# Hagtaril/HiddenPose

Hardware: AMD Instinct MI355X
Metric: samples/sec (128x128x512 meas) fwd+bwd (higher is better)
Workload: dtype f32; 1 GPU; NlosPose train step (fwd+L2Joint+BCEDice loss+bwd+Adam), 128x128x512 transients, batch 4/GPU, fp32, random-init weights, weight gradients of the 3^3 / 4^3 convolutions (and of small 1^3 ones) on a second stream; global_batch=4, world_size=1, parallelism=dp1

## Files before the change

### hiddenpose_amd/_lib.py

```python
from __future__ import annotations

import ctypes as C
import os
import threading

_PKG = os.path.dirname(os.path.abspath(__file__))
LIB_PATH = os.path.join(_PKG, "libhiddenpose_hip.so")

_lock = threading.Lock()
_lib = None


class HiddenPoseHipError(RuntimeError):
    pass


_vp, _fp, _i, _sz, _d = C.c_void_p, C.c_void_p, C.c_int, C.c_size_t, C.c_double
SIGNATURES = {
    "hp_version": (_i, []),
    "hp_last_error_string": (C.c_char_p, []),
    "hp_profile_enable": (_i, [_i]),
    "hp_profile_reset": (_i, []),
    "hp_profile_count": (_i, []),
    "hp_profile_get": (_i, [_i, C.c_char_p, _i, C.POINTER(C.c_int64), C.POINTER(C.c_double)]),
# ... 7 lines not shown
    "hp_lct_plan_create_mode": (_i, [C.POINTER(_vp), _i, _i, _d, _d, _i, _i, _i]),
    "hp_lct_plan_destroy": (_i, [_vp]),
    "hp_laplacian5_forward": (_i, [_fp, _fp, _fp, C.c_long, _i, _i, _i, _vp]),
    "hp_laplacian5_backward": (_i, [_fp, _fp, _fp, C.c_long, _i, _i, _i, _vp]),
    "hp_lct_workspace_bytes": (_sz, [_vp, _i]),
    "hp_lct_forward": (_i, [_vp, _fp, _fp, _i, _vp, _sz, _vp]),
    "hp_lct_backward": (_i, [_vp, _fp, _fp, _i, _vp, _sz, _vp]),
    "hp_lct_plan_get_invpsf": (_i, [_vp, _vp, _vp]),
    "hp_conv3d_packed_weight_elems": (_sz, [_vp]),
    "hp_conv3d_pack_weight": (_i, [_vp, _fp, _fp, _fp, _vp]),
    "hp_conv3d_unpack_wgrad": (_i, [_vp, _fp, _fp, _vp]),
    "hp_conv3d_forward": (_i, [_vp, _fp, _fp, _fp, _fp, _vp, _vp]),
    "hp_conv3d_backward_data": (_i, [_vp, _fp, _fp, _fp, _fp, _vp]),
    "hp_conv3d_backward_data_masked": (_i, [_vp, _fp, _fp, _fp, _fp, _vp, _vp]),
    "hp_conv3d_backward_data_bnsums": (_i, [_vp, _fp, _fp, _fp, _fp, _vp, _fp, _fp, _fp, _fp, _fp, _i, _vp, _vp, C.POINTER(C.c_int), _vp]),
    "hp_bn_backward_presummed": (_i, [_fp, _fp, _fp, C.c_long, _i, _fp, _fp, _fp, _fp, _i, _i, _fp, _fp, _vp, _vp, _vp, _i, _vp]),
    "hp_conv3d_backward_weight": (_i, [_vp, _fp, _fp, _fp, _vp]),
    "hp_conv3d_backward_weight_split": (_i, [_vp, C.POINTER(C.c_long), C.POINTER(C.c_long)]),
    "hp_bn_train_finalize": (_i, [_vp, C.c_long, _i, C.c_float, C.c_float, _fp, _fp, _fp, _fp, _vp]),
    "hp_bn_train_finalize_counted": (_i, [_vp, C.c_long, _i, C.c_float, C.c_float, _fp, _fp, _fp, _fp, _vp, _vp]),
    "hp_bn_eval_stats": (_i, [_fp, _fp, _i, C.c_float, _fp, _fp, _vp]),
    "hp_bn_apply": (_i, [_fp, _fp, _fp, C.c_long, _i, _fp, _fp, _fp, _fp, _i, _vp, _i, _vp]),
    "hp_bn_apply_res_bn": (_i, [_fp, _fp, _fp, C.c_long, _i, _fp, _fp, _fp, _fp, _i, _vp, _fp, _fp, _fp, _fp, _i, _vp]),
    "hp_cast_f32_to_bf16": (_i, [_fp, _vp, C.c_long, _vp]),
    "hp_cast_bf16_to_f32": (_i, [_vp, _fp, C.c_long, _vp]),
    "hp_bn_backward_workspace_bytes": (_sz, [_i]),
    "hp_bn_backward_dual": (_i, [_fp, _vp, C.c_long, _i, _fp, _fp, _fp, _fp, _fp, _i, _fp, _fp, _fp, _fp, _fp, _fp, _fp, _i,
                                 _fp, _fp, _vp, _i, _vp]),
    "hp_bn_backward": (_i, [_fp, _fp, _fp, _fp, _fp, C.c_long, _i, _fp, _fp, _fp, _fp, _i, _i, _fp, _fp, _vp, _vp, _i, _vp]),
    "hp_maxpool3d_k3s2_forward": (_i, [_fp, _fp, _i, _i, _i, _i, _i, _vp]),
# ... 194 lines not shown
```

### hiddenpose_amd/csrc/conv_kernels.hip

```cpp
#include <algorithm>
#include <cstdlib>
#include <cstring>
#include <mutex>
#include <type_traits>
#include <vector>

#include "hp_internal.h"

namespace hp {

using f32x16 = __attribute__((ext_vector_type(16))) float;
using bf16x8 = __attribute__((ext_vector_type(8))) __bf16;
using bf16x4 = __attribute__((ext_vector_type(4))) __bf16;
using bf16x2 = __attribute__((ext_vector_type(2))) __bf16;
using f32x2 = __attribute__((ext_vector_type(2))) float;
using s16x4 = __attribute__((ext_vector_type(4))) short;

__device__ __forceinline__ bf16x4 to_bf16x4(const float4 v) {
  const bf16x2 lo = __builtin_convertvector((f32x2){v.x, v.y}, bf16x2);
  const bf16x2 hi = __builtin_convertvector((f32x2){v.z, v.w}, bf16x2);
  return (bf16x4){lo[0], lo[1], hi[0], hi[1]};
}

enum IgemmMode { MODE_CONV = 0, MODE_DECONV = 1, MODE_DGRAD_S2K3 = 2, MODE_STEM = 3 };
// ... 27 lines not shown
    x = (int)(u & (unsigned)(g.gw - 1));
    y = (int)((u >> g.sw) & (unsigned)(g.gh - 1));
    z = (int)((u >> (g.sw + g.sh)) & (unsigned)(g.gd - 1));
    b = (int)(u >> (g.sw + g.sh + g.sd));
  } else {
    long t = m;
    x = (int)(t % g.gw);
    t /= g.gw;
    y = (int)(t % g.gh);
    t /= g.gh;
    z = (int)(t % g.gd);
    b = (int)(t / g.gd);
  }
}

template <int NP>
__device__ __forceinline__ void split_bf16(const float4 v, bf16x4 (&out)[NP]) {
  float4 r = v;
#pragma unroll
  for (int p = 0; p < NP; ++p) {
    out[p] = to_bf16x4(r);
    if (p + 1 < NP) {
      r.x -= (float)out[p][0];
      r.y -= (float)out[p][1];
      r.z -= (float)out[p][2];
      r.w -= (float)out[p][3];
    }
  }
}
template <int NP>
// ... 60 lines not shown
    dx = pw ? 1 - jw : 0;
    widx = (kd * 3 + kh) * 3 + kw;
  }
}

template <int BN>
struct TileCfg {
  static constexpr int WN = BN >= 64 ? 2 : 1;
  static constexpr int WM = 4 / WN;
  static constexpr int TM = BM / (WM * 32);
  static constexpr int TN = BN / (WN * 32);
};

__device__ __attribute__((aligned(256))) unsigned int g_zero_row[64];

template <int BN, bool STEM, bool STATS, int NP, bool XH = false, bool GL = false, bool BL = false, int BNS = 0>
__global__ __launch_bounds__(CT, (NP == 0 && BN == 128) ? 3 : 1) void k_igemm(const void* __restrict__ Xv, const float* __restrict__ Wp,
                                              const float* __restrict__ bias, void* __restrict__ Y,
                                              double* __restrict__ stats, const void* __restrict__ addend,
                                              const unsigned char* __restrict__ amask, IgemmGeom g) {
  const float* const X = (const float*)Xv;
  constexpr bool IOH = NP == 1;
  auto ld_x4 = [&](long off) -> float4 {
    if constexpr (IOH) return hp_ld4(Xv, off, g.xh);
    else return *(const float4*)(X + off);
  };
  auto ld_a4 = [&](long off) -> float4 {
    if constexpr (IOH) return hp_ld4(addend, off, g.ah);
    else return *(const float4*)((const float*)addend + off);
  };
  auto ld_a1 = [&](long off) -> float {
// ... 2 lines not shown
  };
  auto st_y4 = [&](long off, float4 v) {
    if constexpr (IOH) hp_st4(Y, off, v, g.yh);
    else *(float4*)((float*)Y + off) = v;
  };
  auto st_y1 = [&](long off, float v) {
    if constexpr (IOH) hp_st1(Y, off, v, g.yh);
    else ((float*)Y)[off] = v;
  };
  using C = TileCfg<BN>;
  constexpr bool BF = NP > 0;
  constexpr int NPL = NP > 0 ? NP : 1;
  static_assert(!XH || (NP == 1 && !STEM), "bf16-storage tiles: single bf16 plane, not the stem");
  static_assert(!GL || (XH && BN >= 64), "direct-to-LDS tiles: bf16 storage, 64 or 128 columns");
  static_assert(!BL || (!XH && !STEM), "buffer-load tiles: fp32 tensors in memory (any arithmetic), not the stem");
  constexpr int BKT = XH ? 64 : BK;
  constexpr int LDX = GL ? BKT : BKT + 8;
  constexpr int EPL = XH ? 8 : 4;
  constexpr int ARENA0 = (BM + BN) * LDK > NP * (BM + BN) * LDH / 2 ? (BM + BN) * LDK : NP * (BM + BN) * LDH / 2;
  constexpr int ARENA1 = XH && (BM + BN) * LDX / 2 > ARENA0 ? (BM + BN) * LDX / 2 : ARENA0;
  constexpr int GLBUF = (BM + BN) * 64;
  constexpr int ARENA = GL ? GLBUF : ARENA1;
  __shared__ __attribute__((aligned(16))) float smem[ARENA];
  float* const As = smem;
  float* const Bs = smem + BM * LDK;
  __bf16* const Ah = (__bf16*)smem;
  __bf16* const Bh = Ah + NPL * BM * (XH ? LDX : LDH);
  __shared__ float red[STATS ? 2 * BN * C::WM : 1];
  const int tid = threadIdx.x, lane = tid & 63, wave = tid >> 6;
  const int wm = wave / C::WN, wn = wave % C::WN;
  const int cls = blockIdx.z;
  unsigned mt_idx = blockIdx.x, nt_idx = blockIdx.y;
  if (g.tn > 0) {
    const unsigned i = blockIdx.x >> 3;
    nt_idx = i % (unsigned)g.tn;
    mt_idx = g.slab > 0 ? (blockIdx.x & 7u) * (unsigned)g.slab + i / (unsigned)g.tn : (i / (unsigned)g.tn) * 8u + (blockIdx.x & 7u);
    if ((long)mt_idx * BM >= g.M) return;
  } else if (g.slab > 0) {
    mt_idx = (blockIdx.x & 7u) * (unsigned)g.slab + (blockIdx.x >> 3);
    if ((long)mt_idx * BM >= g.M) return;
  }
  const long m0 = (long)mt_idx * BM;
  const int n0 = nt_idx * BN;
  const int pd = (cls >> 2) & 1, ph = (cls >> 1) & 1, pw = cls & 1;

  const int kq0 = tid & 7, r0 = tid >> 3;
  const int kq = GL ? (kq0 ^ ((r0 >> 1) & 7)) : kq0;
  int rb[4], rz[4], ry[4], rx[4];
  bool rv[4];
#pragma unroll
  for (int i = 0; i < 4; ++i) {
    const long m = m0 + r0 + 32 * i;
    rv[i] = m < g.M;
    grid_coords(g, rv[i] ? m : 0, rb[i], rz[i], ry[i], rx[i]);
    rx[i] *= g.s;
    ry[i] *= g.s;
    rz[i] *= g.s;
  }
  const int ntaps = STEM ? 1 : class_ntaps(g, cls);
  const int kpt = XH ? (g.Cin + BKT - 1) / BKT : g.kpt;
  const int KT = ntaps * kpt;

  long rowoff[4], wrow[BN / 32];
  unsigned long long vmask[4];
  bool wvalid[BN / 32];
#pragma unroll
  for (int i = 0; i < 4; ++i) {
    rowoff[i] = ((((long)rb[i] * g.Di + rz[i]) * g.Hi + ry[i]) * g.Wi + rx[i]) * g.Cin + kq * EPL;
    vmask[i] = 0ull;
  }
  if constexpr (!STEM) {
    for (int t = ntaps - 1; t >= 0; --t) {
      int dz, dy, dx, widx;
      tap_info(g, cls, t, dz, dy, dx, widx);
#pragma unroll
      for (int i = 0; i < 4; ++i) {
        const bool ok = rv[i] && (unsigned)(rz[i] + dz) < (unsigned)g.Di && (unsigned)(ry[i] + dy) < (unsigned)g.Hi &&
                        (unsigned)(rx[i] + dx) < (unsigned)g.Wi;
        vmask[i] = (vmask[i] << 1) | (ok ? 1ull : 0ull);
      }
    }
  }
#pragma unroll
  for (int i = 0; i < BN / 32; ++i) {
    const int n = n0 + r0 + 32 * i;
    wvalid[i] = n < g.Nout;
    const int nsrc = g.geglu ? ((n & 64) ? (g.Nout >> 1) + ((n >> 7) << 6) + (n & 63) : ((n >> 7) << 6) + (n & 63)) : n;
    wrow[i] = (long)nsrc * g.Cin + kq * EPL;
  }

  constexpr unsigned OOB = 0x80000000u;
  long rowbase = 0;
  unsigned xrow32[4] = {0u, 0u, 0u, 0u}, xvoff[4] = {OOB, OOB, OOB, OOB}, wvoff[BN / 32];
  long min_xoff = 0;
  if constexpr (BL) {
    for (int t = 0; t < ntaps; ++t) {
      int dz, dy, dx, widx;
      tap_info(g, cls, t, dz, dy, dx, widx);
      const long xo = (((long)dz * g.Hi + dy) * g.Wi + dx) * g.Cin;
      min_xoff = (t == 0 || xo < min_xoff) ? xo : min_xoff;
    }
    int b0, z0, y0, x0;
    grid_coords(g, m0 < g.M ? m0 : 0, b0, z0, y0, x0);
    rowbase = ((((long)b0 * g.Di + z0 * g.s) * g.Hi + y0 * g.s) * g.Wi + x0 * g.s) * g.Cin;
#pragma unroll
    for (int i = 0; i < 4; ++i) xrow32[i] = rv[i] ? (unsigned)((rowoff[i] - rowbase) * 4) : OOB;
#pragma unroll
    for (int i = 0; i < BN / 32; ++i) wvoff[i] = wvalid[i] ? (unsigned)(wrow[i] * 4) : OOB;
  }
  const __amdgpu_buffer_rsrc_t xrs = __builtin_amdgcn_make_buffer_rsrc(
      (void*)(X + (rowbase + min_xoff)), 0, hp_extent((long)g.B * g.Di * g.Hi * g.Wi * g.Cin, rowbase + min_xoff, 4), 0x00020000);
  const __amdgpu_buffer_rsrc_t wrs = __builtin_amdgcn_make_buffer_rsrc((void*)Wp, 0, hp_extent(g.welems, 0, 4), 0x00020000);
  float4 ra[4], rbw[BN / 32];
  uint4 ra8[XH ? 4 : 1];
  float4 rbw2[XH ? BN / 32 : 1];
  uint4 rb8[XH ? BN / 32 : 1];
  int ld_tap = 0, ld_ci = 0;
  long ld_xoff = 0, ld_woff = 0;
  unsigned ninv_lo[4] = {0u, 0u, 0u, 0u}, ninv_hi[4] = {0u, 0u, 0u, 0u};
// ... 4 lines not shown
      ninv_hi[i] = ~(unsigned)(vmask[i] >> 32);
    }
  }
  auto tap_offsets = [&](int t) {
    int dz, dy, dx, widx;
    tap_info(g, cls, t, dz, dy, dx, widx);
    ld_xoff = (((long)dz * g.Hi + dy) * g.Wi + dx) * g.Cin;
    ld_woff = (long)widx * g.Nout * g.Cin;
    if constexpr (BL) {
      const unsigned tb = (unsigned)t & 31u;
#pragma unroll
      for (int i = 0; i < 4; ++i)
        xvoff[i] = xrow32[i] | (__builtin_amdgcn_ubfe(t < 32 ? ninv_lo[i] : ninv_hi[i], tb, 1u) << 31);
    }
  };
  if (!STEM) tap_offsets(0);
  auto load_tile = [&](int kt) {
    if constexpr (STEM) {
      const int kbase = kt * BK + kq * 4;
#pragma unroll
      for (int i = 0; i < 4; ++i) {
        float v[4];
#pragma unroll
        for (int j = 0; j < 4; ++j) {
          const int kk = kbase + j;
          const int a = kk / 49, b = (kk / 7) % 7, c = kk % 7;
          const int z = rz[i] + a - 3, y = ry[i] + b - 3, x = rx[i] + c - 3;
          const bool ok = rv[i] && kk < 343 && (unsigned)z < (unsigned)g.Di && (unsigned)y < (unsigned)g.Hi &&
                          (unsigned)x < (unsigned)g.Wi;
          v[j] = ok ? X[(unsigned)(((rb[i] * g.Di + z) * g.Hi + y) * g.Wi + x)] : 0.f;
        }
// ... 34 lines not shown
        for (int i = 0; i < BN / 32; ++i) rbw[i] = __builtin_bit_cast(float4, __builtin_amdgcn_raw_buffer_load_b128(wrs, wvoff[i], ws, 0));
      } else {
#pragma unroll
        for (int i = 0; i < 4; ++i)
          ra[i] = (cok && (vmask[i] & 1ull)) ? ld_x4(xb + rowoff[i]) : make_float4(0, 0, 0, 0);
#pragma unroll
        for (int i = 0; i < BN / 32; ++i)
          rbw[i] = (cok && wvalid[i]) ? *(const float4*)(wb + wrow[i]) : make_float4(0, 0, 0, 0);
      }
      if (++ld_ci == kpt) {
        ld_ci = 0;
        if constexpr (!BL) {
#pragma unroll
          for (int i = 0; i < 4; ++i) vmask[i] >>= 1;
        }
        if (++ld_tap < ntaps) tap_offsets(ld_tap);
      }
    }
  };
  unsigned lds_a[4], lds_b[BN / 32];
#pragma unroll
  for (int i = 0; i < 4; ++i) {
    lds_a[i] = (unsigned)(((r0 + 32 * i) * LDK + kq * 4) * 4);
    asm volatile("" : "+v"(lds_a[i]));
  }
#pragma unroll
  for (int i = 0; i < BN / 32; ++i) {
    lds_b[i] = (unsigned)((BM * LDK + (r0 + 32 * i) * LDK + kq * 4) * 4);
    asm volatile("" : "+v"(lds_b[i]));
  }
  auto store_tile = [&]() {
// ... 180 lines not shown
      }
      __syncthreads();
    }
    if (kt + 1 < KT) {
      store_tile();
      __syncthreads();
    }
  }

  const bool dense_out = (g.os == 1 && g.gd == g.Do && g.gh == g.Ho && g.gw == g.Wo);
  if constexpr (BN >= 64) {
    constexpr int LDO = BN + 4, Q = BN / 4;
    static_assert(64 * LDO <= ARENA, "staging tile must fit the arena");
    static_assert(C::WM == 2 && C::TM == 2, "epilogue assumes 2 waves x 2 MFMA tiles along M");
    const bool vec_ok = (g.Nout & 3) == 0;
    const bool fast = !IOH && dense_out && vec_ok && m0 + BM <= g.M && n0 + BN <= g.Nout && !g.geglu;
    const long tile_el = m0 * g.Nout + n0;
    const long y_el = g.M * g.Nout;
    const unsigned y_rec = hp_extent(y_el, tile_el, 4);
    const __amdgpu_buffer_rsrc_t yrs = __builtin_amdgcn_make_buffer_rsrc((void*)((float*)Y + tile_el), 0, y_rec, 0x00020000);
    const __amdgpu_buffer_rsrc_t ars =
        __builtin_amdgcn_make_buffer_rsrc((void*)((addend ? (const float*)addend : (const float*)Y) + tile_el), 0, y_rec, 0x00020000);
    const __amdgpu_buffer_rsrc_t mrs = __builtin_amdgcn_make_buffer_rsrc(
        (void*)((amask ? amask : (const unsigned char*)Y) + (tile_el >> 2)), 0, hp_extent(y_el >> 2, tile_el >> 2, 1), 0x00020000);
    constexpr int RPK = CT / Q;
    const int r_l = tid / Q, q_l = tid % Q;
    const unsigned vo = (unsigned)((r_l * g.Nout + 4 * q_l) * 4);
    float4 bv = make_float4(0, 0, 0, 0);
    if (fast && bias) bv = *(const float4*)(bias + n0 + 4 * q_l);
    [[maybe_unused]] __amdgpu_buffer_rsrc_t zrs = yrs, bmrs = mrs;
    [[maybe_unused]] float4 b_m = make_float4(0, 0, 0, 0), b_r = b_m, b_sc = b_m, b_sh = b_m, b_s = b_m, b_d = b_m;
    if constexpr (BNS) {
      zrs = __builtin_amdgcn_make_buffer_rsrc((void*)(g.bn_z + tile_el), 0, y_rec, 0x00020000);
      if constexpr (BNS == 2)
        bmrs = __builtin_amdgcn_make_buffer_rsrc((void*)(g.bn_mask + (tile_el >> 2)), 0, hp_extent(y_el >> 2, tile_el >> 2, 1), 0x00020000);
      b_m = *(const float4*)(g.bn_mean + n0 + 4 * q_l);
      b_r = *(const float4*)(g.bn_rstd + n0 + 4 * q_l);
      if (BNS == 1 && g.bn_relu) {
        const float4 ga = *(const float4*)(g.bn_gamma + n0 + 4 * q_l), be = *(const float4*)(g.bn_beta + n0 + 4 * q_l);
        b_sc = make_float4(b_r.x * ga.x, b_r.y * ga.y, b_r.z * ga.z, b_r.w * ga.w);
        b_sh = make_float4(be.x - b_m.x * b_sc.x, be.y - b_m.y * b_sc.y, be.z - b_m.z * b_sc.z, be.w - b_m.w * b_sc.w);
      }
// ... 5 lines not shown
      for (int r = 0; r < 16; ++r) {
        const int rl = wm * 32 + (r & 3) + 8 * (r >> 2) + 4 * (lane >> 5);
#pragma unroll
        for (int j = 0; j < C::TN; ++j) smem[rl * LDO + wn * C::TN * 32 + j * 32 + (lane & 31)] = acc[h][j][r];
      }
      constexpr int K2 = (64 * Q) / CT;
      float4 avb[K2];
      unsigned mkb[K2];
      [[maybe_unused]] float4 zvb[BNS ? K2 : 1];
      [[maybe_unused]] unsigned bmb[BNS == 2 ? K2 : 1];
      if constexpr (BNS) {
#pragma unroll
        for (int k2 = 0; k2 < K2; ++k2) {
          const int rowc = k2 * RPK;
          const unsigned so = (unsigned)(((rowc >> 5) * (C::TM * 32) + h * 32 + (rowc & 31)) * g.Nout * 4);
          zvb[k2] = __builtin_bit_cast(float4, __builtin_amdgcn_raw_buffer_load_b128(zrs, vo, so, 0));
          if constexpr (BNS == 2) bmb[k2] = (unsigned)__builtin_amdgcn_raw_buffer_load_b8(bmrs, vo >> 4, so >> 4, 0);
        }
      }
      if (fast && addend) {
#pragma unroll
        for (int k2 = 0; k2 < K2; ++k2) {
          const int rowc = k2 * RPK;
          const unsigned so = (unsigned)(((rowc >> 5) * (C::TM * 32) + h * 32 + (rowc & 31)) * g.Nout * 4);
          avb[k2] = __builtin_bit_cast(float4, __builtin_amdgcn_raw_buffer_load_b128(ars, vo, so, 0));
        }
        if (amask) {
#pragma unroll
          for (int k2 = 0; k2 < K2; ++k2) {
            const int rowc = k2 * RPK;
            const unsigned so = (unsigned)(((rowc >> 5) * (C::TM * 32) + h * 32 + (rowc & 31)) * g.Nout * 4);
            mkb[k2] = __builtin_amdgcn_raw_buffer_load_b8(mrs, vo >> 4, so >> 4, 0);
          }
        }
      }
      __syncthreads();
      if constexpr (BN == 128) {
        if (g.geglu && dense_out && m0 + BM <= g.M && n0 + BN <= g.Nout) {
          constexpr int QH = Q / 2;
          float* const yg = (float*)Y + m0 * (long)(g.Nout / 2) + n0 / 2;
          float4 bv4 = make_float4(0, 0, 0, 0), bg4 = bv4;
          const int qg = tid % QH, rg = tid / QH;
          if (bias) {
            bv4 = *(const float4*)(bias + n0 / 2 + 4 * qg);
            bg4 = *(const float4*)(bias + g.Nout / 2 + n0 / 2 + 4 * qg);
          }
// ... 3 lines not shown
            const int row64 = rg + k2 * (CT / QH);
            const int trow = (row64 >> 5) * (C::TM * 32) + h * 32 + (row64 & 31);
            float4 v = *(const float4*)(smem + row64 * LDO + 4 * qg), gt = *(const float4*)(smem + row64 * LDO + BN / 2 + 4 * qg);
            v.x += bv4.x; v.y += bv4.y; v.z += bv4.z; v.w += bv4.w;
            gt.x += bg4.x; gt.y += bg4.y; gt.z += bg4.z; gt.w += bg4.w;
            *(float4*)(yg + (long)trow * (g.Nout / 2) + 4 * qg) = make_float4(gl(v.x, gt.x), gl(v.y, gt.y), gl(v.z, gt.z), gl(v.w, gt.w));
          }
          continue;
        }
      }
      if (fast) {
#pragma unroll
        for (int k2 = 0; k2 < K2; ++k2) {
          const int rowc = k2 * RPK;
          const int trow_c = (rowc >> 5) * (C::TM * 32) + h * 32 + (rowc & 31);
          const unsigned so = (unsigned)(trow_c * g.Nout * 4);
          float4 v = *(const float4*)(smem + (r_l + rowc) * LDO + 4 * q_l);
          v.x += bv.x; v.y += bv.y; v.z += bv.z; v.w += bv.w;
          if (addend) {
            float4 av = avb[k2];
            if (amask) {
              const unsigned mk = mkb[k2];
              av.x = (mk & 1u) ? av.x : 0.f;
              av.y = (mk & 2u) ? av.y : 0.f;
              av.z = (mk & 4u) ? av.z : 0.f;
              av.w = (mk & 8u) ? av.w : 0.f;
            }
            v.x += av.x; v.y += av.y; v.z += av.z; v.w += av.w;
          }
          typedef unsigned u32x4 __attribute__((ext_vector_type(4)));
          __builtin_amdgcn_raw_buffer_store_b128(__builtin_bit_cast(u32x4, v), yrs, vo, so, 0);
          if constexpr (BNS) {
            const float4 zz = zvb[k2];
            float4 gg = v;
            if constexpr (BNS == 2) {
              const unsigned bm = bmb[k2];
              gg.x = (bm & 1u) ? v.x : 0.f;
              gg.y = (bm & 2u) ? v.y : 0.f;
              gg.z = (bm & 4u) ? v.z : 0.f;
              gg.w = (bm & 8u) ? v.w : 0.f;
            } else if (g.bn_relu) {
              gg.x = fmaf(zz.x, b_sc.x, b_sh.x) > 0.f ? v.x : 0.f;
              gg.y = fmaf(zz.y, b_sc.y, b_sh.y) > 0.f ? v.y : 0.f;
              gg.z = fmaf(zz.z, b_sc.z, b_sh.z) > 0.f ? v.z : 0.f;
              gg.w = fmaf(zz.w, b_sc.w, b_sh.w) > 0.f ? v.w : 0.f;
            }
// ... 1760 lines not shown
    p.wgrad = f;
    p.wgrad_tapsum = 64;
    p.dgrad = IgemmGeom{MODE_CONV, d.B, Do, Ho, Wo, d.Cout, d.Di, d.Hi, d.Wi, d.Cin, d.Di, d.Hi, d.Wi, 1,
                        4, 2, 1, 0, (long)d.B * d.Di * d.Hi * d.Wi, d.Cout / 32};
    p.dgrad_classes = 1;
  }
  HP_REQUIRE((long)d.B * d.Di * d.Hi * d.Wi * (d.transposed ? 8 : 1) < (1l << 31), "conv: more than 2^31 voxels per tensor");
  set_shifts(p.fwd);
  set_shifts(p.dgrad);
  set_shifts(p.wgrad);
  p.fwd.welems = p.wgrad.welems = p.stem ? (long)d.Cout * ((343 + 31) / 32 * 32) : (long)d.Cout * d.Cin * k * k * k;
  p.dgrad.welems = (long)d.Cout * d.Cin * k * k * k;
  return HP_OK;
}

template <bool STEM, bool STATS, int NP, bool XH = false>
static void launch_igemm_bn(const IgemmGeom& g, int classes, const void* X, const float* W, const float* bias, void* Y,
                            double* stats, const void* addend, const unsigned char* amask, hipStream_t st) {
  if constexpr (NP == 1 && !STEM && !XH) {
    if (g.xh && g.Cin % 64 == 0) return launch_igemm_bn<STEM, STATS, NP, true>(g, classes, X, W, bias, Y, stats, addend, amask, st);
  }
  const unsigned mt = (unsigned)((g.M + BM - 1) / BM);
  static const bool gl_on = !(getenv("HP_IGEMM_GL") && atoi(getenv("HP_IGEMM_GL")) == 0);
  const bool gl = XH && g.wh && gl_on;
  static const bool bl_on = !(getenv("HP_IGEMM_BL") && atoi(getenv("HP_IGEMM_BL")) == 0);
  const bool bl = !XH && !g.xh && !g.wh && !STEM && bl_on && g.Cin % 32 == 0 && (long)g.Nout * g.Cin * class_ntaps(g, 0) * 4 * (g.mode == MODE_DECONV ? 8 : 1) < (1l << 31);
  static const bool slab_on = !(getenv("HP_IGEMM_SLAB") && atoi(getenv("HP_IGEMM_SLAB")) == 0);
  if (slab_on && g.Nout <= 64) {
    IgemmGeom gs = g;
    gs.slab = (int)((mt + 7) / 8);
    const dim3 grid((mt + 7) / 8 * 8, 1, classes);
    if constexpr (!XH && !STEM) {
      if (bl && g.Nout > 32) {
        hipLaunchKernelGGL((k_igemm<64, false, STATS, NP, false, false, true>), grid, dim3(CT), 0, st, X, W, bias, Y, stats, addend, amask, gs);
        return;
      }
    }
  }
  if (g.Nout > 64) {
    const unsigned tn = (unsigned)((g.Nout + 127) / 128);
    IgemmGeom gg = g;
    gg.tn = tn > 1 ? (int)tn : 0;
    gg.slab = slab_on ? (int)((mt + 7) / 8) : 0;
    const dim3 grid = (tn > 1 || gg.slab) ? dim3((mt + 7) / 8 * 8 * (tn > 1 ? tn : 1), 1, classes) : dim3(mt, 1, classes);
    if constexpr (XH) {
      if (gl) {
        hipLaunchKernelGGL((k_igemm<128, STEM, STATS, NP, true, true>), grid, dim3(CT), 0, st, X, W, bias, Y, stats, addend, amask, gg);
        return;
      }
    }
    if constexpr (!XH && !STEM) {
      if (bl) {
        hipLaunchKernelGGL((k_igemm<128, false, STATS, NP, false, false, true>), grid, dim3(CT), 0, st, X, W, bias, Y, stats, addend, amask, gg);
        return;
      }
    }
    hipLaunchKernelGGL((k_igemm<128, STEM, STATS, NP, XH>), grid, dim3(CT), 0, st, X, W, bias, Y, stats, addend, amask, gg);
  } else if (g.Nout > 32) {
    if constexpr (XH) {
      if (gl) {
        hipLaunchKernelGGL((k_igemm<64, STEM, STATS, NP, true, true>), dim3(mt, 1, classes), dim3(CT), 0, st, X, W, bias, Y, stats, addend, amask, g);
        return;
      }
    }
    if constexpr (!XH && !STEM) {
      if (bl) {
        hipLaunchKernelGGL((k_igemm<64, false, STATS, NP, false, false, true>), dim3(mt, 1, classes), dim3(CT), 0, st, X, W, bias, Y, stats, addend, amask, g);
        return;
      }
    }
    hipLaunchKernelGGL((k_igemm<64, STEM, STATS, NP, XH>), dim3(mt, 1, classes), dim3(CT), 0, st, X, W, bias, Y, stats, addend, amask, g);
  } else {
    hipLaunchKernelGGL((k_igemm<32, STEM, STATS, NP, XH>), dim3(mt, 1, classes), dim3(CT), 0, st, X, W, bias, Y, stats, addend, amask, g);
  }
}

template <int NP>
static void launch_igemm_p(const IgemmGeom& g, int classes, bool stem, const void* X, const float* W, const float* bias,
                           void* Y, double* stats, const void* addend, const unsigned char* amask, hipStream_t st) {
  if (stem) {
    if (stats) launch_igemm_bn<true, true, NP>(g, classes, X, W, bias, Y, stats, addend, amask, st);
// ... 6 lines not shown

static void launch_igemm(const IgemmGeom& g, int classes, bool stem, int planes, const void* X, const float* W,
                         const float* bias, void* Y, double* stats, const void* addend, hipStream_t st,
                         const unsigned char* amask = nullptr) {
  switch (planes) {
    case 1: launch_igemm_p<1>(g, classes, stem, X, W, bias, Y, stats, addend, amask, st); break;
    case 2: launch_igemm_p<2>(g, classes, stem, X, W, bias, Y, stats, addend, amask, st); break;
    case 3: launch_igemm_p<3>(g, classes, stem, X, W, bias, Y, stats, addend, amask, st); break;
    default: launch_igemm_p<0>(g, classes, stem, X, W, bias, Y, stats, addend, amask, st); break;
  }
}

}

using namespace hp;

extern "C" size_t hp_conv3d_packed_weight_elems(const hp_conv_desc* d) {
  if (!d) return 0;
  if (!d->transposed && d->Cin == 1 && d->k == 7) return (size_t)d->Cout * ((343 + 31) / 32 * 32);
  return (size_t)d->Cout * d->Cin * d->k * d->k * d->k;
}

extern "C" int hp_conv3d_pack_weight(const hp_conv_desc* d, const float* w_torch, void* w_fwd_v, void* w_dgrad_v,
                                     void* stream) {
  float* const w_fwd = (float*)w_fwd_v;
  float* const w_dgrad = (float*)w_dgrad_v;
  HP_REQUIRE(d && w_torch, "hp_conv3d_pack_weight: null argument");
  ConvPlan p;
  int rc = make_plan(*d, p);
  if (rc) return rc;
// ... 121 lines not shown
  }
  HP_CHECK_HIP(hipGetLastError());
  return HP_OK;
}

static bool launch_igemm_bns(const IgemmGeom& g, const void* X, const float* W, void* Y, const void* addend,
                             const unsigned char* amask, hipStream_t st) {
  const bool dense_out = g.os == 1 && g.gd == g.Do && g.gh == g.Ho && g.gw == g.Wo;
  if (g.mode != MODE_CONV || !dense_out || g.M % BM != 0 || g.Nout <= 32 || g.Nout % (g.Nout > 64 ? 128 : 64) != 0 || g.xh || g.yh ||
      g.wh || g.ah)
    return false;
  const unsigned mt = (unsigned)(g.M / BM);
  static const bool bl_on = !(getenv("HP_IGEMM_BL") && atoi(getenv("HP_IGEMM_BL")) == 0);
  static const bool slab_on = !(getenv("HP_IGEMM_SLAB") && atoi(getenv("HP_IGEMM_SLAB")) == 0);
  const bool bl = bl_on && g.Cin % 32 == 0 && (long)g.Nout * g.Cin * class_ntaps(g, 0) * 4 < (1l << 31);
  IgemmGeom gg = g;
  gg.slab = slab_on ? (int)((mt + 7) / 8) : 0;
#define HP_BNS_LAUNCH(BN_, BL_)                                                                                                     \
  do {                                                                                                                             \
    if (g.bn_mask)                                                                                                                 \
      hipLaunchKernelGGL((k_igemm<BN_, false, false, 0, false, false, BL_, 2>), grid, dim3(CT), 0, st, X, W, nullptr, Y, nullptr,   \
                         addend, amask, gg);                                                                                       \
    else                                                                                                                           \
      hipLaunchKernelGGL((k_igemm<BN_, false, false, 0, false, false, BL_, 1>), grid, dim3(CT), 0, st, X, W, nullptr, Y, nullptr,   \
                         addend, amask, gg);                                                                                       \
  } while (0)
  if (g.Nout <= 64) {
    const dim3 grid = gg.slab ? dim3((mt + 7) / 8 * 8, 1, 1) : dim3(mt, 1, 1);
    if (bl) HP_BNS_LAUNCH(64, true);
    else HP_BNS_LAUNCH(64, false);
    return true;
  }
  const unsigned tn = (unsigned)(g.Nout / 128);
  gg.tn = tn > 1 ? (int)tn : 0;
  const dim3 grid = (tn > 1 || gg.slab) ? dim3((mt + 7) / 8 * 8 * (tn > 1 ? tn : 1), 1, 1) : dim3(mt, 1, 1);
  if (bl) HP_BNS_LAUNCH(128, true);
  else HP_BNS_LAUNCH(128, false);
#undef HP_BNS_LAUNCH
  return true;
}

extern "C" int hp_conv3d_backward_data_bnsums(const hp_conv_desc* d, const void* dy, const float* w_dgrad, void* dx, const void* addend,
                                              const unsigned char* addend_mask, const float* z, const float* mean,
                                              const float* rstd, const float* gamma, const float* beta, int relu,
                                              const unsigned char* relu_mask, double* sums, int* fused, void* stream) {
  HP_REQUIRE(d && dy && w_dgrad && dx && z && mean && rstd && sums && fused && (!relu || relu_mask || (gamma && beta)),
             "hp_conv3d_backward_data_bnsums: null argument");
  *fused = 0;
  ConvPlan p;
  int rc = make_plan(*d, p);
  if (rc) return rc;
  hipStream_t st = (hipStream_t)stream;
  if (p.planes == 0 && !p.stem && !p.dgrad_zero_fill && d->io == 0 && p.dgrad_classes == 1 &&
// ... 283 lines not shown
```

### hiddenpose_amd/hip_ops.py

```python
from __future__ import annotations

import os

import torch
import torch.nn.functional as F

HIP_STAGES = {"feature_extraction", "lct_forward", "lct_backward", "normalize_feature", "unet3d", "posenet3d_50",
              "softmax_integral", "weighted_mse", "bce_dice"}
ATEN_STAGES = {"Adam"}
from .optimizer import hip_optimizer_selected as _hip_optimizer_selected

if _hip_optimizer_selected():
    HIP_STAGES, ATEN_STAGES = HIP_STAGES | {"Adam"}, set()


def _need_cuda(x: torch.Tensor, what: str) -> None:
    if not x.is_cuda:
        from ._lib import HiddenPoseHipError

        raise HiddenPoseHipError(f"{what}: tensor is on {x.device}; this package has no CPU path")


import ctypes as _C

# ... 539 lines not shown

def set_conv_precision(name: str) -> str:
    global _conv_precision
    if name not in _PRECISIONS:
        raise ValueError(f"conv precision must be one of {sorted(_PRECISIONS)}, got {name!r}")
    global _conv_precision_name, _act_bf16
    prev = get_conv_precision()
    _conv_precision = _PRECISIONS[name]
    _conv_precision_name = name
    _act_bf16 = name == "bf16s"
    return prev


def get_conv_precision() -> str:
    return _conv_precision_name


def _desc(x_cl, cout, k, stride, pad, transposed):
    b, d, h, w, cin = x_cl.shape
    return _lib.ConvDesc(b, d, h, w, cin, cout, k, stride, pad, 1 if transposed else 0, _conv_precision)


def _out_dims(desc):
    if desc.transposed:
        return 2 * desc.Di, 2 * desc.Hi, 2 * desc.Wi
    f = lambda n: (n + 2 * desc.pad - desc.k) // desc.stride + 1
    return f(desc.Di), f(desc.Hi), f(desc.Wi)


def _same_as_packed(desc):
# ... 825 lines not shown
```

### include/hiddenpose_hip.h

```cpp
#ifndef HIDDENPOSE_HIP_H
#define HIDDENPOSE_HIP_H

#include <stddef.h>
#include <stdint.h>

#ifdef __cplusplus
extern "C" {
#endif

typedef enum hp_status {
  HP_OK = 0,
  HP_ERR_BAD_ARG = -1,
  HP_ERR_UNSUPPORTED = -2,
  HP_ERR_HIP = -3,
  HP_ERR_WORKSPACE = -4,
  HP_ERR_NO_DEVICE = -5
} hp_status;

int hp_version(void);
const char* hp_last_error_string(void);

int hp_profile_enable(int on);
int hp_profile_reset(void);
int hp_profile_count(void);
// ... 48 lines not shown
#define HP_IO_Y_BF16 2
#define HP_IO_DY_BF16 4
#define HP_IO_DX_BF16 8
#define HP_IO_W_BF16 16

size_t hp_conv3d_packed_weight_elems(const hp_conv_desc* d);
int hp_conv3d_pack_weight(const hp_conv_desc* d, const float* w_torch, void* w_fwd, void* w_dgrad, void* stream);
int hp_conv3d_unpack_wgrad(const hp_conv_desc* d, const float* dw_packed, float* dw_torch, void* stream);
#define HP_STATS_SLOTS 32
int hp_conv3d_forward(const hp_conv_desc* d, const void* x, const float* w_fwd, const float* bias, void* y,
                      double* stats, void* stream);
int hp_conv3d_backward_data(const hp_conv_desc* d, const void* dy, const float* w_dgrad, void* dx,
                            const void* addend, void* stream);
int hp_conv3d_backward_data_masked(const hp_conv_desc* d, const void* dy, const float* w_dgrad, void* dx,
                                   const void* addend, const unsigned char* addend_mask, void* stream);
int hp_conv3d_backward_data_bnsums(const hp_conv_desc* d, const void* dy, const float* w_dgrad, void* dx, const void* addend,
                                   const unsigned char* addend_mask, const float* z, const float* mean, const float* rstd,
                                   const float* gamma, const float* beta, int relu, const unsigned char* relu_mask, double* sums,
                                   int* fused, void* stream);
int hp_conv3d_backward_weight(const hp_conv_desc* d, const void* x, const void* dy, float* dw_packed, void* stream);
int hp_conv3d_backward_weight_split(const hp_conv_desc* d, long* msplit, long* chunk_rows);

#define HP_BN_ACT_BF16 1
#define HP_BN_DY_BF16 2
#define HP_BN_DZ_BF16 4
#define HP_BN_Z_BF16 8
int hp_bn_train_finalize(const double* stats, long M, int C, float eps, float momentum, float* mean, float* rstd,
                         float* running_mean, float* running_var, void* stream);
int hp_bn_train_finalize_counted(const double* stats, long M, int C, float eps, float momentum, float* mean, float* rstd,
                                 float* running_mean, float* running_var, long long* num_batches_tracked, void* stream);
// ... 269 lines not shown
```

Baseline: 8.780 samples/s.

## Reorder implicit-GEMM rows by boundary face to skip all-padding taps

Adds a 'face order' mode for exact-fp32 buffer-load implicit-GEMM conv tiles. Output rows are remapped so each tile holds rows from a single H/W boundary class (corners, edges, interior), and the tile ORs its rows' tap-validity masks to iterate only the taps that touch real data. The epilogue scatters results through per-row offsets kept in shared memory. A heuristic enables it by default for large stride-1 k3 flipped convs and stride-2 k3 dgrad, trading extra index math, a block sync and scattered stores for fewer K-tiles on boundary tiles.

```diff
diff --git a/hiddenpose_amd/_lib.py b/hiddenpose_amd/_lib.py
--- a/hiddenpose_amd/_lib.py
+++ b/hiddenpose_amd/_lib.py
@@ -45,6 +45,8 @@
     "hp_conv3d_backward_data": (_i, [_vp, _fp, _fp, _fp, _fp, _vp]),
     "hp_conv3d_backward_data_masked": (_i, [_vp, _fp, _fp, _fp, _fp, _vp, _vp]),
     "hp_conv3d_backward_data_bnsums": (_i, [_vp, _fp, _fp, _fp, _fp, _vp, _fp, _fp, _fp, _fp, _fp, _i, _vp, _vp, C.POINTER(C.c_int), _vp]),
+    "hp_conv_set_face_order": (_i, [_i]),
+    "hp_conv_face_order_plan": (_i, [_vp, _i]),
     "hp_bn_backward_presummed": (_i, [_fp, _fp, _fp, C.c_long, _i, _fp, _fp, _fp, _fp, _i, _i, _fp, _fp, _vp, _vp, _vp, _i, _vp]),
     "hp_conv3d_backward_weight": (_i, [_vp, _fp, _fp, _fp, _vp]),
     "hp_conv3d_backward_weight_split": (_i, [_vp, C.POINTER(C.c_long), C.POINTER(C.c_long)]),
diff --git a/hiddenpose_amd/csrc/conv_kernels.hip b/hiddenpose_amd/csrc/conv_kernels.hip
--- a/hiddenpose_amd/csrc/conv_kernels.hip
+++ b/hiddenpose_amd/csrc/conv_kernels.hip
@@ -65,6 +65,34 @@
   }
 }
 
+__device__ __forceinline__ void face_coords(const IgemmGeom& g, unsigned m, int& b, int& z, int& y, int& x) {
+  const unsigned bz = (unsigned)(g.B * g.gd);
+  unsigned start = 0u, sel_start = 0u;
+  int sel = 0;
+#pragma unroll
+  for (int c = 0; c < 9; ++c) {
+    const unsigned ny = (c / 3 == 1) ? (unsigned)(g.gh - 2) : 1u, nx = (c % 3 == 1) ? (unsigned)(g.gw - 2) : 1u;
+    if (m >= start) {
+      sel = c;
+      sel_start = start;
+    }
+    start += bz * ny * nx;
+  }
+  const int cy = sel / 3, cx = sel - 3 * cy;
+  const unsigned ny = cy == 1 ? (unsigned)(g.gh - 2) : 1u, nx = cx == 1 ? (unsigned)(g.gw - 2) : 1u;
+  const int y0 = cy == 0 ? 0 : cy == 1 ? 1 : g.gh - 1, x0 = cx == 0 ? 0 : cx == 1 ? 1 : g.gw - 1;
+  unsigned t = m - sel_start;
+  unsigned q = t / nx;
+  x = x0 + (int)(t - q * nx);
+  t = q;
+  q = t / ny;
+  y = y0 + (int)(t - q * ny);
+  t = q;
+  q = t / (unsigned)g.gd;
+  z = (int)(t - q * (unsigned)g.gd);
+  b = (int)q;
+}
+
 template <int NP>
 __device__ __forceinline__ void split_bf16(const float4 v, bf16x4 (&out)[NP]) {
   float4 r = v;
@@ -155,7 +183,7 @@
 
 __device__ __attribute__((aligned(256))) unsigned int g_zero_row[64];
 
-template <int BN, bool STEM, bool STATS, int NP, bool XH = false, bool GL = false, bool BL = false, int BNS = 0>
+template <int BN, bool STEM, bool STATS, int NP, bool XH = false, bool GL = false, bool BL = false, int BNS = 0, bool FO = false>
 __global__ __launch_bounds__(CT, (NP == 0 && BN == 128) ? 3 : 1) void k_igemm(const void* __restrict__ Xv, const float* __restrict__ Wp,
                                               const float* __restrict__ bias, void* __restrict__ Y,
                                               double* __restrict__ stats, const void* __restrict__ addend,
@@ -188,6 +216,7 @@
   static_assert(!XH || (NP == 1 && !STEM), "bf16-storage tiles: single bf16 plane, not the stem");
   static_assert(!GL || (XH && BN >= 64), "direct-to-LDS tiles: bf16 storage, 64 or 128 columns");
   static_assert(!BL || (!XH && !STEM), "buffer-load tiles: fp32 tensors in memory (any arithmetic), not the stem");
+  static_assert(!FO || (BL && NP == 0 && BN >= 64), "face order: exact-fp32 buffer-load tiles of 64 / 128 columns");
   constexpr int BKT = XH ? 64 : BK;
   constexpr int LDX = GL ? BKT : BKT + 8;
   constexpr int EPL = XH ? 8 : 4;
@@ -201,6 +230,8 @@
   __bf16* const Ah = (__bf16*)smem;
   __bf16* const Bh = Ah + NPL * BM * (XH ? LDX : LDH);
   __shared__ float red[STATS ? 2 * BN * C::WM : 1];
+  [[maybe_unused]] __shared__ unsigned fo_orow[FO ? BM : 1];
+  [[maybe_unused]] __shared__ unsigned long long fo_or;
   const int tid = threadIdx.x, lane = tid & 63, wave = tid >> 6;
   const int wm = wave / C::WN, wn = wave % C::WN;
   const int cls = blockIdx.z;
@@ -226,14 +257,21 @@
   for (int i = 0; i < 4; ++i) {
     const long m = m0 + r0 + 32 * i;
     rv[i] = m < g.M;
-    grid_coords(g, rv[i] ? m : 0, rb[i], rz[i], ry[i], rx[i]);
+    if constexpr (FO) {
+      face_coords(g, rv[i] ? (unsigned)m : 0u, rb[i], rz[i], ry[i], rx[i]);
+      if (kq0 == 0)
+        fo_orow[r0 + 32 * i] =
+            rv[i] ? (unsigned)(((rb[i] * g.Do + rz[i] * g.os + pd) * g.Ho + ry[i] * g.os + ph) * g.Wo + rx[i] * g.os + pw) * (unsigned)(g.Nout * 4)
+                  : 0x80000000u;
+    } else {
+      grid_coords(g, rv[i] ? m : 0, rb[i], rz[i], ry[i], rx[i]);
+    }
     rx[i] *= g.s;
     ry[i] *= g.s;
     rz[i] *= g.s;
   }
   const int ntaps = STEM ? 1 : class_ntaps(g, cls);
   const int kpt = XH ? (g.Cin + BKT - 1) / BKT : g.kpt;
-  const int KT = ntaps * kpt;
 
   long rowoff[4], wrow[BN / 32];
   unsigned long long vmask[4];
@@ -255,6 +293,17 @@
       }
     }
   }
+  [[maybe_unused]] unsigned long long fo_rem = 0ull;
+  if constexpr (FO) {
+    if (tid == 0) fo_or = 0ull;
+    __syncthreads();
+    if (kq0 == 0) atomicOr(&fo_or, vmask[0] | vmask[1] | vmask[2] | vmask[3]);
+    __syncthreads();
+    const unsigned long long o = fo_or;
+    fo_rem = ((unsigned long long)(unsigned)__builtin_amdgcn_readfirstlane((int)(unsigned)(o >> 32)) << 32) |
+             (unsigned)__builtin_amdgcn_readfirstlane((int)(unsigned)o);
+  }
+  const int KT = FO ? __builtin_popcountll(fo_rem) * kpt : ntaps * kpt;
 #pragma unroll
   for (int i = 0; i < BN / 32; ++i) {
     const int n = n0 + r0 + 32 * i;
@@ -274,9 +323,11 @@
       const long xo = (((long)dz * g.Hi + dy) * g.Wi + dx) * g.Cin;
       min_xoff = (t == 0 || xo < min_xoff) ? xo : min_xoff;
     }
-    int b0, z0, y0, x0;
-    grid_coords(g, m0 < g.M ? m0 : 0, b0, z0, y0, x0);
-    rowbase = ((((long)b0 * g.Di + z0 * g.s) * g.Hi + y0 * g.s) * g.Wi + x0 * g.s) * g.Cin;
+    if constexpr (!FO) {
+      int b0, z0, y0, x0;
+      grid_coords(g, m0 < g.M ? m0 : 0, b0, z0, y0, x0);
+      rowbase = ((((long)b0 * g.Di + z0 * g.s) * g.Hi + y0 * g.s) * g.Wi + x0 * g.s) * g.Cin;
+    }
 #pragma unroll
     for (int i = 0; i < 4; ++i) xrow32[i] = rv[i] ? (unsigned)((rowoff[i] - rowbase) * 4) : OOB;
 #pragma unroll
@@ -311,7 +362,12 @@
         xvoff[i] = xrow32[i] | (__builtin_amdgcn_ubfe(t < 32 ? ninv_lo[i] : ninv_hi[i], tb, 1u) << 31);
     }
   };
-  if (!STEM) tap_offsets(0);
+  if constexpr (FO) {
+    ld_tap = fo_rem ? __builtin_ctzll(fo_rem) : 0;
+    tap_offsets(ld_tap);
+  } else if (!STEM) {
+    tap_offsets(0);
+  }
   auto load_tile = [&](int kt) {
     if constexpr (STEM) {
       const int kbase = kt * BK + kq * 4;
@@ -376,7 +432,15 @@
 #pragma unroll
           for (int i = 0; i < 4; ++i) vmask[i] >>= 1;
         }
-        if (++ld_tap < ntaps) tap_offsets(ld_tap);
+        if constexpr (FO) {
+          fo_rem &= fo_rem - 1ull;
+          if (fo_rem) {
+            ld_tap = __builtin_ctzll(fo_rem);
+            tap_offsets(ld_tap);
+          }
+        } else {
+          if (++ld_tap < ntaps) tap_offsets(ld_tap);
+        }
       }
     }
   };
@@ -587,9 +651,9 @@
     static_assert(64 * LDO <= ARENA, "staging tile must fit the arena");
     static_assert(C::WM == 2 && C::TM == 2, "epilogue assumes 2 waves x 2 MFMA tiles along M");
     const bool vec_ok = (g.Nout & 3) == 0;
-    const bool fast = !IOH && dense_out && vec_ok && m0 + BM <= g.M && n0 + BN <= g.Nout && !g.geglu;
-    const long tile_el = m0 * g.Nout + n0;
-    const long y_el = g.M * g.Nout;
+    const bool fast = FO || (!IOH && dense_out && vec_ok && m0 + BM <= g.M && n0 + BN <= g.Nout && !g.geglu);
+    const long tile_el = FO ? (long)n0 : m0 * g.Nout + n0;
+    const long y_el = FO ? (long)g.B * g.Do * g.Ho * g.Wo * g.Nout : g.M * g.Nout;
     const unsigned y_rec = hp_extent(y_el, tile_el, 4);
     const __amdgpu_buffer_rsrc_t yrs = __builtin_amdgcn_make_buffer_rsrc((void*)((float*)Y + tile_el), 0, y_rec, 0x00020000);
     const __amdgpu_buffer_rsrc_t ars =
@@ -599,6 +663,12 @@
     constexpr int RPK = CT / Q;
     const int r_l = tid / Q, q_l = tid % Q;
     const unsigned vo = (unsigned)((r_l * g.Nout + 4 * q_l) * 4);
+    [[maybe_unused]] auto fo_offsets = [&](int h, int k2, unsigned& rvo, unsigned& rso, unsigned& rmo) {
+      const int rowc = k2 * RPK;
+      rvo = fo_orow[r_l + (rowc >> 5) * (C::TM * 32) + h * 32 + (rowc & 31)] + (unsigned)(16 * q_l);
+      rso = 0u;
+      rmo = (rvo >> 4) | (rvo & 0x80000000u);
+    };
     float4 bv = make_float4(0, 0, 0, 0);
     if (fast && bias) bv = *(const float4*)(bias + n0 + 4 * q_l);
     [[maybe_unused]] __amdgpu_buffer_rsrc_t zrs = yrs, bmrs = mrs;
@@ -634,6 +704,13 @@
         for (int k2 = 0; k2 < K2; ++k2) {
           const int rowc = k2 * RPK;
           const unsigned so = (unsigned)(((rowc >> 5) * (C::TM * 32) + h * 32 + (rowc & 31)) * g.Nout * 4);
+          if constexpr (FO) {
+            unsigned rvo, rso, rmo;
+            fo_offsets(h, k2, rvo, rso, rmo);
+            zvb[k2] = __builtin_bit_cast(float4, __builtin_amdgcn_raw_buffer_load_b128(zrs, rvo, rso, 0));
+            if constexpr (BNS == 2) bmb[k2] = (unsigned)__builtin_amdgcn_raw_buffer_load_b8(bmrs, rmo, rso, 0);
+            continue;
+          }
           zvb[k2] = __builtin_bit_cast(float4, __builtin_amdgcn_raw_buffer_load_b128(zrs, vo, so, 0));
           if constexpr (BNS == 2) bmb[k2] = (unsigned)__builtin_amdgcn_raw_buffer_load_b8(bmrs, vo >> 4, so >> 4, 0);
         }
@@ -643,6 +720,12 @@
         for (int k2 = 0; k2 < K2; ++k2) {
           const int rowc = k2 * RPK;
           const unsigned so = (unsigned)(((rowc >> 5) * (C::TM * 32) + h * 32 + (rowc & 31)) * g.Nout * 4);
+          if constexpr (FO) {
+            unsigned rvo, rso, rmo;
+            fo_offsets(h, k2, rvo, rso, rmo);
+            avb[k2] = __builtin_bit_cast(float4, __builtin_amdgcn_raw_buffer_load_b128(ars, rvo, rso, 0));
+            continue;
+          }
           avb[k2] = __builtin_bit_cast(float4, __builtin_amdgcn_raw_buffer_load_b128(ars, vo, so, 0));
         }
         if (amask) {
@@ -650,6 +733,12 @@
           for (int k2 = 0; k2 < K2; ++k2) {
             const int rowc = k2 * RPK;
             const unsigned so = (unsigned)(((rowc >> 5) * (C::TM * 32) + h * 32 + (rowc & 31)) * g.Nout * 4);
+            if constexpr (FO) {
+              unsigned rvo, rso, rmo;
+              fo_offsets(h, k2, rvo, rso, rmo);
+              mkb[k2] = __builtin_amdgcn_raw_buffer_load_b8(mrs, rmo, rso, 0);
+              continue;
+            }
             mkb[k2] = __builtin_amdgcn_raw_buffer_load_b8(mrs, vo >> 4, so >> 4, 0);
           }
         }
@@ -683,7 +772,11 @@
         for (int k2 = 0; k2 < K2; ++k2) {
           const int rowc = k2 * RPK;
           const int trow_c = (rowc >> 5) * (C::TM * 32) + h * 32 + (rowc & 31);
-          const unsigned so = (unsigned)(trow_c * g.Nout * 4);
+          unsigned so = (unsigned)(trow_c * g.Nout * 4), rvo = vo;
+          if constexpr (FO) {
+            unsigned rmo;
+            fo_offsets(h, k2, rvo, so, rmo);
+          }
           float4 v = *(const float4*)(smem + (r_l + rowc) * LDO + 4 * q_l);
           v.x += bv.x; v.y += bv.y; v.z += bv.z; v.w += bv.w;
           if (addend) {
@@ -698,7 +791,7 @@
             v.x += av.x; v.y += av.y; v.z += av.z; v.w += av.w;
           }
           typedef unsigned u32x4 __attribute__((ext_vector_type(4)));
-          __builtin_amdgcn_raw_buffer_store_b128(__builtin_bit_cast(u32x4, v), yrs, vo, so, 0);
+          __builtin_amdgcn_raw_buffer_store_b128(__builtin_bit_cast(u32x4, v), yrs, rvo, so, 0);
           if constexpr (BNS) {
             const float4 zz = zvb[k2];
             float4 gg = v;
@@ -2489,6 +2582,45 @@
   return HP_OK;
 }
 
+static int g_face_order = [] {
+  const char* e = getenv("HP_IGEMM_FACE_ORDER");
+  const int v = e ? atoi(e) : 1;
+  return v < 0 || v > 2 ? 1 : v;
+}();
+
+static bool face_order_supported(const IgemmGeom& g) {
+  if (g.mode == MODE_STEM || class_ntaps(g, 7) <= 1 || g.geglu || g.xh || g.yh || g.wh || g.ah) return false;
+  if (g.gh < 2 || g.gw < 2 || g.Cin % 32 != 0 || g.Nout % (g.Nout > 64 ? 128 : 64) != 0) return false;
+  const long xb = (long)g.B * g.Di * g.Hi * g.Wi * g.Cin * 4, yb = (long)g.B * g.Do * g.Ho * g.Wo * g.Nout * 4;
+  return xb < (1l << 31) && yb < (1l << 31) && g.M < (1l << 31);
+}
+
+static double face_order_share(const IgemmGeom& g) {
+  auto axis = [&](int n) -> double {
+    if (g.mode == MODE_DECONV || g.mode == MODE_DGRAD_S2K3) return 1.0 - 1.0 / (2.0 * n);
+    if (g.k == 3 && g.s == 1) return 1.0 - 2.0 / (3.0 * n);
+    if (g.k == 4 && g.s == 2) return 1.0 - 2.0 / (4.0 * n);
+    if (g.k == 3 && g.s == 2) return 1.0 - 1.0 / (3.0 * n);
+    return 1.0;
+  };
+  return 1.0 - axis(g.gh) * axis(g.gw);
+}
+
+constexpr double FO_MIN_SAVED_KTILES = 3.0;
+constexpr long FO_MIN_WORKGROUPS_S1 = 1024, FO_MIN_WORKGROUPS_S2 = 4096;
+static bool face_order_rule(const IgemmGeom& g, bool bns) {
+  if (bns || face_order_share(g) * class_ntaps(g, 7) * g.kpt < FO_MIN_SAVED_KTILES) return false;
+  const long wgs = ((g.M + BM - 1) / BM) * ((g.Nout + 127) / 128);
+  if (g.mode == MODE_CONV && g.k == 3 && g.s == 1 && g.flip) return wgs >= FO_MIN_WORKGROUPS_S1;
+  if (g.mode == MODE_DGRAD_S2K3) return 8 * wgs >= FO_MIN_WORKGROUPS_S2;
+  return false;
+}
+
+static bool face_order_use(const IgemmGeom& g, bool bns = false) {
+  if (g_face_order == 0 || !face_order_supported(g)) return false;
+  return g_face_order == 2 || face_order_rule(g, bns);
+}
+
 template <bool STEM, bool STATS, int NP, bool XH = false>
 static void launch_igemm_bn(const IgemmGeom& g, int classes, const void* X, const float* W, const float* bias, void* Y,
                             double* stats, const void* addend, const unsigned char* amask, hipStream_t st) {
@@ -2507,6 +2639,12 @@
     const dim3 grid((mt + 7) / 8 * 8, 1, classes);
     if constexpr (!XH && !STEM) {
       if (bl && g.Nout > 32) {
+        if constexpr (NP == 0) {
+          if (face_order_use(g)) {
+            hipLaunchKernelGGL((k_igemm<64, false, STATS, 0, false, false, true, 0, true>), grid, dim3(CT), 0, st, X, W, bias, Y, stats, addend, amask, gs);
+            return;
+          }
+        }
         hipLaunchKernelGGL((k_igemm<64, false, STATS, NP, false, false, true>), grid, dim3(CT), 0, st, X, W, bias, Y, stats, addend, amask, gs);
         return;
       }
@@ -2526,6 +2664,12 @@
     }
     if constexpr (!XH && !STEM) {
       if (bl) {
+        if constexpr (NP == 0) {
+          if (face_order_use(g)) {
+            hipLaunchKernelGGL((k_igemm<128, false, STATS, 0, false, false, true, 0, true>), grid, dim3(CT), 0, st, X, W, bias, Y, stats, addend, amask, gg);
+            return;
+          }
+        }
         hipLaunchKernelGGL((k_igemm<128, false, STATS, NP, false, false, true>), grid, dim3(CT), 0, st, X, W, bias, Y, stats, addend, amask, gg);
         return;
       }
@@ -2540,6 +2684,12 @@
     }
     if constexpr (!XH && !STEM) {
       if (bl) {
+        if constexpr (NP == 0) {
+          if (face_order_use(g)) {
+            hipLaunchKernelGGL((k_igemm<64, false, STATS, 0, false, false, true, 0, true>), dim3(mt, 1, classes), dim3(CT), 0, st, X, W, bias, Y, stats, addend, amask, g);
+            return;
+          }
+        }
         hipLaunchKernelGGL((k_igemm<64, false, STATS, NP, false, false, true>), dim3(mt, 1, classes), dim3(CT), 0, st, X, W, bias, Y, stats, addend, amask, g);
         return;
       }
@@ -2576,6 +2726,23 @@
 }
 
 using namespace hp;
+
+extern "C" int hp_conv_set_face_order(int mode) {
+  HP_REQUIRE(mode >= 0 && mode <= 2, "hp_conv_set_face_order: mode 0, 1 or 2 (got %d)", mode);
+  g_face_order = mode;
+  return HP_OK;
+}
+
+extern "C" int hp_conv_face_order_plan(const hp_conv_desc* d, int dgrad) {
+  if (!d) return -1;
+  ConvPlan p;
+  if (make_plan(*d, p)) return -1;
+  const IgemmGeom& g = dgrad ? p.dgrad : p.fwd;
+  static const bool bl_on = !(getenv("HP_IGEMM_BL") && atoi(getenv("HP_IGEMM_BL")) == 0);
+  const bool bl = p.planes == 0 && d->io == 0 && !p.stem && bl_on && g.Nout > 32 &&
+                  (long)g.Nout * g.Cin * class_ntaps(g, 0) * 4 * (g.mode == MODE_DECONV ? 8 : 1) < (1l << 31);
+  return bl && face_order_use(g) ? 1 : 0;
+}
 
 extern "C" size_t hp_conv3d_packed_weight_elems(const hp_conv_desc* d) {
   if (!d) return 0;
@@ -2727,8 +2894,18 @@
   static const bool bl_on = !(getenv("HP_IGEMM_BL") && atoi(getenv("HP_IGEMM_BL")) == 0);
   static const bool slab_on = !(getenv("HP_IGEMM_SLAB") && atoi(getenv("HP_IGEMM_SLAB")) == 0);
   const bool bl = bl_on && g.Cin % 32 == 0 && (long)g.Nout * g.Cin * class_ntaps(g, 0) * 4 < (1l << 31);
+  const bool fo = bl && face_order_use(g, true);
   IgemmGeom gg = g;
   gg.slab = slab_on ? (int)((mt + 7) / 8) : 0;
+#define HP_BNS_LAUNCH_FO(BN_)                                                                                                       \
+  do {                                                                                                                             \
+    if (g.bn_mask)                                                                                                                 \
+      hipLaunchKernelGGL((k_igemm<BN_, false, false, 0, false, false, true, 2, true>), grid, dim3(CT), 0, st, X, W, nullptr, Y,    \
+                         nullptr, addend, amask, gg);                                                                              \
+    else                                                                                                                           \
+      hipLaunchKernelGGL((k_igemm<BN_, false, false, 0, false, false, true, 1, true>), grid, dim3(CT), 0, st, X, W, nullptr, Y,    \
+                         nullptr, addend, amask, gg);                                                                              \
+  } while (0)
 #define HP_BNS_LAUNCH(BN_, BL_)                                                                                                     \
   do {                                                                                                                             \
     if (g.bn_mask)                                                                                                                 \
@@ -2740,16 +2917,19 @@
   } while (0)
   if (g.Nout <= 64) {
     const dim3 grid = gg.slab ? dim3((mt + 7) / 8 * 8, 1, 1) : dim3(mt, 1, 1);
-    if (bl) HP_BNS_LAUNCH(64, true);
+    if (bl && fo) HP_BNS_LAUNCH_FO(64);
+    else if (bl) HP_BNS_LAUNCH(64, true);
     else HP_BNS_LAUNCH(64, false);
     return true;
   }
   const unsigned tn = (unsigned)(g.Nout / 128);
   gg.tn = tn > 1 ? (int)tn : 0;
   const dim3 grid = (tn > 1 || gg.slab) ? dim3((mt + 7) / 8 * 8 * (tn > 1 ? tn : 1), 1, 1) : dim3(mt, 1, 1);
-  if (bl) HP_BNS_LAUNCH(128, true);
+  if (bl && fo) HP_BNS_LAUNCH_FO(128);
+  else if (bl) HP_BNS_LAUNCH(128, true);
   else HP_BNS_LAUNCH(128, false);
 #undef HP_BNS_LAUNCH
+#undef HP_BNS_LAUNCH_FO
   return true;
 }
 
diff --git a/hiddenpose_amd/hip_ops.py b/hiddenpose_amd/hip_ops.py
--- a/hiddenpose_amd/hip_ops.py
+++ b/hiddenpose_amd/hip_ops.py
@@ -577,6 +577,10 @@
 
 def get_conv_precision() -> str:
     return _conv_precision_name
+
+
+def set_conv_face_order(mode: int) -> None:
+    _lib.check(_lib.lib().hp_conv_set_face_order(int(mode)), "hp_conv_set_face_order")
 
 
 def _desc(x_cl, cout, k, stride, pad, transposed):
diff --git a/include/hiddenpose_hip.h b/include/hiddenpose_hip.h
--- a/include/hiddenpose_hip.h
+++ b/include/hiddenpose_hip.h
@@ -86,6 +86,8 @@
                             const void* addend, void* stream);
 int hp_conv3d_backward_data_masked(const hp_conv_desc* d, const void* dy, const float* w_dgrad, void* dx,
                                    const void* addend, const unsigned char* addend_mask, void* stream);
+int hp_conv_set_face_order(int mode);
+int hp_conv_face_order_plan(const hp_conv_desc* d, int dgrad);
 int hp_conv3d_backward_data_bnsums(const hp_conv_desc* d, const void* dy, const float* w_dgrad, void* dx, const void* addend,
                                    const unsigned char* addend_mask, const float* z, const float* mean, const float* rstd,
                                    const float* gamma, const float* beta, int relu, const unsigned char* relu_mask, double* sums,
```

Result: no change. 8.769 samples/s (-0.1%).
